# pzimbrod/fem-glass-tempering

Measured on AMD Instinct MI355X. Metric: DOF-updates/sec (coupled thermo-visco time step, 3D CG1 hex), higher is better.
Workload: dtype f64; 1 GPU; C4 3D plate CG1/CG1 400x400x50 hex (8200851 T-dofs), dt 0.1, coupled 6-term Prony; parallelism=single GPU, one partition (no communication), output=none (reference writes VTX/XDMF every step), krylov_form=PETSc KSPCG, geometric-multigrid V-cycle preconditioner, preconditioner=gmg, visco_fields=state (T, Tf, Tf_partial, phi, xi, s_tilde, sigma_tilde, sigma)

## Files before the change

fem-glass-tempering_amd/csrc/tv_context.cpp:

```cpp
#include <cstdlib>

#include "tv_ctx.h"

namespace tv {

static std::mutex g_err_mu;
static std::string g_err;

void set_global_error(const std::string& m) {
  std::lock_guard<std::mutex> lk(g_err_mu);
  g_err = m;
}

void axis_coefs(const std::vector<double>& X, int first, int count, std::vector<double>& out) {
  const int n = (int)X.size();
  out.assign((size_t)count * C_NCOEF, 0.0);
  for (int q = 0; q < count; ++q) {
    const int i = first + q;
    double* c = &out[(size_t)q * C_NCOEF];
    if (n == 1) {
      c[C_MDI] = 1.0;
      continue;
    }
    const double hlo = (i > 0) ? X[i] - X[i - 1] : 0.0;
// ... 1098 lines not shown
    output_release(c->out, set);
    return c->fail(TV_ERR_HIP, std::string("output gather: ") + hipGetErrorString(e));
  }
  std::string err;
  if (!output_submit(c->out, set, t, c->stream, err)) return c->fail(TV_ERR_STATE, "output: " + err);
  return TV_OK;
}


int tv_output_close(void* ctx) {
  Ctx* c = static_cast<Ctx*>(ctx);
  if (!c) return TV_ERR_ARG;
  if (!c->out) return TV_OK;
  hipSetDevice(c->device);
  const std::string e = output_destroy(c->out);
  c->out = nullptr;
  c->out_fields.clear();
  if (!e.empty()) return c->fail(TV_ERR_STATE, "output: " + e);
  return TV_OK;
}


int tv_set_dirichlet(void* ctx, int enable, double value) {
  Ctx* c = static_cast<Ctx*>(ctx);
  if (!c) return TV_ERR_ARG;
  if (c->O.model_mode != TV_MODEL_PAPER)
    return c->fail(TV_ERR_STATE, "Dirichlet condition: only with model_mode = TV_MODEL_PAPER (the reference's "
                                 "own path cannot run, ThermoViscoProblem.py:236-243)");
  if (enable && c->amg_on)
    return c->fail(TV_ERR_STATE, "Dirichlet condition: not with TV_PC_AMG (Jacobi or the box multigrid)");
  hipSetDevice(c->device);
  c->dir_on = enable != 0;
  c->dir_value = value;
  if (c->dir_on && c->fam_T == TV_CG && !c->dB) {
    const size_t nb = sizeof(double) * (size_t)std::max<int64_t>(1, c->nT);
    HIPC(tv_dev_alloc(&c->dB, nb, kMemDoubles));
    HIPC(tv_dev_alloc(&c->dtmp, nb, kMemDoubles));
    HIPC(hipMemsetAsync(c->dtmp, 0, nb, c->stream));
    HIPC(hipStreamSynchronize(c->stream));
  }
  return TV_OK;
}


int tv_sync(void* ctx) {
  Ctx* c = static_cast<Ctx*>(ctx);
  if (!c) return TV_ERR_ARG;
  HIPC(hipStreamSynchronize(c->stream));
  return TV_OK;
}


int tv_get_options(void* ctx, tv_options* out) {
  Ctx* c = static_cast<Ctx*>(ctx);
  if (!c || !out) return TV_ERR_ARG;
  *out = c->O;
  return TV_OK;
}


int tv_set_newton_tolerances(void* ctx, double rtol, double atol, int max_it, int error_on_nonconvergence) {
  Ctx* c = static_cast<Ctx*>(ctx);
  if (!c) return TV_ERR_ARG;
  if (!(rtol >= 0.0) || !(atol >= 0.0) || max_it < 1)
    return c->fail(TV_ERR_ARG, "Newton tolerances: rtol >= 0, atol >= 0 and max_it >= 1");
  c->O.newton_rtol = rtol;
// ... 21 lines not shown
```

fem-glass-tempering_amd/csrc/tv_ctx.h:

```cpp
#pragma once
#include <rccl/rccl.h>

#include <algorithm>
#include <array>
#include <cmath>
#include <cstdio>
#include <cstring>
#include <memory>
#include <mutex>
#include <string>
#include <vector>

#include "tv_internal.h"

namespace tv {

struct FieldInfo {
  double* ptr = nullptr;
  void* base = nullptr;
  int bs = 1;
  int space = 0;
  bool alloc = false;
};

struct MgLevel {
  CgGrid g{};
  std::vector<double> X[3];
  int64_t n = 0;
  double omega = 0.0;
  double *T = nullptr, *b = nullptr, *x = nullptr, *w = nullptr, *dinv = nullptr;
  MgXfer xf{};
  double* coef[3] = {nullptr, nullptr, nullptr};
  int64_t* bnodes = nullptr;
  double* ffbuf[2] = {nullptr, nullptr};
  std::vector<void*> bufs;
  bool dinv_interior = false;
  bool dist = false;
  int first2 = 0;
  int inj0 = 0, inj1 = 0;
  double* mask = nullptr;
  RRArgs rr{};
};

struct AmgLevel {
  int64_t n = 0;
  Sell A, P, R;
  UmGrid sg{};
  bool geo0 = false;
  int64_t gfine[3] = {0, 0, 0}, gcoarse[3] = {0, 0, 0};
  int64_t a_nnz = 0, p_nnz = 0, r_nnz = 0;
  double omega = 0.0;
  double *dinv = nullptr, *b = nullptr, *x = nullptr, *w = nullptr;
};

struct Ctx {
  std::string err;
  int device = 0;
  hipStream_t stream = nullptr;
  hipEvent_t ev0 = nullptr, ev1 = nullptr;
  hipEvent_t evp[2] = {nullptr, nullptr};
  hipEvent_t evn[2] = {nullptr, nullptr};
  const double* nrm_dev = nullptr;
  double* ngate = nullptr;
  const double* gate_dev = nullptr;
  const double* solve_gate = nullptr;
  int newton_slot = 0;
  bool newton_first = true;
  bool newton_ahead = true;
  tv_params P{};
  tv_options O{};
  int dim = 1;
  int fam_T = TV_CG, fam_S = TV_CG;
  int perm[3] = {0, -1, -1};
  int n_parts = 1, part = 0;
// ... 152 lines not shown
int allreduce(Ctx* c, double* v, int n);
int reduce_logic(Ctx* c, int n, int W, int kind, int check_done);
int cgs_raxis(const Ctx* c);
int cgs_exchange(Ctx* c, double* wout, const double* fout);
int require_comm(Ctx* c, const char* what);
int refresh_dirty_ghosts(Ctx* c);

void op_residual(Ctx* c, const double* T, const double* Tp, double* F);
void op_diag(Ctx* c, const double* T, double* d, int invert);
void op_japply(Ctx* c, const double* T, const double* x, double* y, double* partials, int* np);
bool op_japply_fused(Ctx* c, const double* T, int* np, const RedTail* tail = nullptr, int it = 0);
PcgState pcg_state_init(const Ctx* c);
int ts_flush(Ctx* c);
CgsBuffers cgs_buffers(Ctx* c, const double* T, int it);
int newton(Ctx* c, int* out_its, int* out_kits, int* out_conv, int step_end = 0, bool* end_queued = nullptr);
int visco(Ctx* c, bool copy_Tprev, const NewtonGate& gate = NewtonGate{});
int queue_newton_norm(Ctx* c, const double* nrm2);
int publish(Ctx* c, void* host_dst, const void* dev_src, size_t bytes);
void launch_bc_mask(Ctx* c, double* dinv);

int mg_setup(Ctx* c);
int mg_prepare(Ctx* c, const double* T);
int mg_dg_weight(Ctx* c, const double* T);
int mg_apply0(Ctx* c, const double* T, const RedTail* tail);
int pcg_solve_mg(Ctx* c, const double* T, int* its, int* reason, bool post = false);
bool mg_next_level(const std::vector<double> (&Xp)[3], double da, bool automatic, std::vector<double> (&Xc)[3],
                   std::vector<char> (&is_c)[3], int coarse[3]);
void mg_axis_tables(const std::vector<double>& Xf, const std::vector<char>& is_c, std::vector<int>& pi,
                    std::vector<double>& pw, std::vector<int>& ri, std::vector<double>& rw);
int mg_level_vectors(Ctx* c, MgLevel& L);
double mg_gershgorin(const std::vector<double> (&X)[3], double dt_alpha);
double mg_omega(double b);
int mg_level(Ctx* c, size_t l);
template <class T>
int mg_upload(Ctx* c, MgLevel& L, const std::vector<T>& h, const T** out) {
  void* p = nullptr;
  HIPC(tv_dev_alloc(&p, sizeof(T) * std::max<size_t>(1, h.size()), mem_kind<T>()));
  L.bufs.push_back(p);
  HIPC(hipMemcpy(p, h.data(), sizeof(T) * h.size(), hipMemcpyHostToDevice));
  *out = static_cast<const T*>(p);
  return TV_OK;
}

int mg_setup_dist(Ctx* c);
int pcg_solve_mg_dist(Ctx* c, const double* T, int* its, int* reason, bool post = false);
int mg_prepare_dist(Ctx* c, const double* T);
void fine_window(const Ctx* c, int64_t* off, int64_t* n);
int mg_apply0_dist(Ctx* c, const double* T, const RedTail* tail);

}
```

fem-glass-tempering_amd/csrc/tv_internal.h:

```cpp
#pragma once
#include <hip/hip_runtime.h>
#include <cstdint>
#include <string>
#include <type_traits>
#include <vector>

#include "tvfem.h"

namespace tv {

constexpr int kWave = 64;
constexpr int kSeg = kWave - 2;
constexpr int kBlock = 256;

enum { kMemDoubles = 0, kMemOther = 1 };
template <class T>
constexpr int mem_kind() {
  return std::is_same<T, double>::value ? kMemDoubles : kMemOther;
}
hipError_t tv_dev_alloc(void** p, size_t bytes, int kind);
hipError_t tv_dev_free(void* p);
template <class T>
inline hipError_t tv_dev_alloc(T** p, size_t bytes, int kind) {
  void* q = nullptr;
// ... 303 lines not shown
  const double* rw[3];
  int aligned;
};
void launch_mg_restrict(const MgXfer& x, const PcgState* st, const double* bf, const double* wf, const FaceAdd* fa,
                        const double* mask, double* bc, const double* dinv_c, double omega_c, double* xc,
                        hipStream_t s);
struct RRAxis {
  const int* f0;
  const double* w;
};
struct RRArgs {
  int on;
  int fn[3], cn[3];
  RRAxis ax[3];
  double da;
  int raxis, nseg, qchunk;
};
constexpr int kRRQMaxChunk = 64;
bool launch_mg_rrestrict(const RRArgs& a, const PcgState* st, const double* b, const double* x, const FaceAdd& fa,
                         double* bc, const double* dinv_c, double omega_c, double* xc, hipStream_t s);
void launch_cg_facet_faces(const CgGrid& g, const double* T, const double* x, const PcgState* st, hipStream_t s);
FaceAdd cg_face_add_all(const CgGrid& g);

struct CoarsePost {
  const double* b;
  const double* w;
  const double* dinv;
  double omega;
  FaceAdd fa;
};
void launch_mg_prolong(const MgXfer& x, const PcgState* st, double* xf, const double* xc, const double* mask,
                       hipStream_t s, const CoarsePost* cp = nullptr);
bool mg_prolong_smooths(const MgXfer& x);
bool mg_restrict_folds_faces(const MgXfer& x);
void launch_mg_jacobi(int64_t n, const PcgState* st, const double* b, const double* w, const FaceAdd* fa,
                      const double* dinv, double omega, double* x, int mode, hipStream_t s);
void launch_mg_inject(const MgXfer& x, const double* Tf, double* Tc, hipStream_t s);
void launch_mg_inject_range(const MgXfer& x, const double* Tf, double* Tc, int k0, int k1, hipStream_t s);
void launch_mg_resid(int64_t n, const PcgState* st, const double* b, double* w, const FaceAdd* fa, const double* mask,
                     hipStream_t s);
void launch_mg_ownmask(int64_t n, int64_t own0, int64_t own1, const double* dinv, double* mask, hipStream_t s);
constexpr int kMgPrepMax = 4;
struct MgPrep {
  int nlev;
  const double* Tbase;
  MgXfer xf[kMgPrepMax];
  double* T[kMgPrepMax];
  double* dinv[kMgPrepMax];
  CgGrid g[kMgPrepMax];
  int64_t off_n[kMgPrepMax + 1];
  int64_t off_b[kMgPrepMax + 1];
};
void launch_mg_prepare(const MgPrep& p, hipStream_t s);
bool cg_uses_march(const CgGrid& g);
void launch_mg_dg_restrict(const DgGrid& g, const PcgState* st, const double* bf, const double* wf, const double* mask,
                           double* bc, const double* dinv_c, double omega_c, double* xc, int kg0, hipStream_t s);
void launch_mg_dg_prolong(const DgGrid& g, const PcgState* st, double* xf, const double* xc, const double* mask,
                          int kg0, hipStream_t s);
void launch_mg_dg_T(const DgGrid& g, const double* Tdg, double* Tcg, int kg0, hipStream_t s);
int launch_mg_pow(int64_t n, const double* dinv, double* y, double* partials, hipStream_t s);
void launch_mg_scale(int64_t n, const double* y, double a, double* x, hipStream_t s);
bool launch_cg_japply_tail(const CgGrid& g, const double* T, const double* x, double* y, const PcgState* st,
                           double* partials, const RedTail* tail, hipStream_t s);
void launch_cg_japply_partial(const CgGrid& g, const double* T, const double* x, double* y, const PcgState* st,
                              hipStream_t s);
void launch_mg_update(int64_t n, const PcgState* st, const double* pA, const double* pB, const double* w,
                      const FaceAdd* fa, const double* dinv, double omega, double* r, double* dx, double* x0,
                      int it_host, int init, hipStream_t s, const double* lag = nullptr,
                      unsigned* counter = nullptr);
void launch_mg_update_cgs(int64_t n, const PcgState* st, const double* u, double* s, const double* z, double* p,
                          double* dx, double* r, const double* dinv, double omega, double* x0, bool first,
                          const double* lag, int lag_kind, unsigned* counter, hipStream_t stream);
int launch_cg_japply_post(const CgGrid& g, const double* T, const double* x, const double* r, const double* dinv,
                          double omega, double* z, const PcgState* st, double* partials, const RedTail* tail,
                          hipStream_t s);
int launch_mg_post(int64_t n, const PcgState* st, const double* x0, const double* r, const double* w,
                   const FaceAdd* fa, const double* dinv, double omega, double* z, double* partials,
                   const RedTail* tail, hipStream_t s);

void launch_pcg_update(int64_t n, PcgState* st, const double* pA, const double* pB, const double* w,
                       const double* dinv, double* dx, double* z, double* partials, hipStream_t s,
                       const RedTail* tail = nullptr, const FaceAdd* fa = nullptr, int it_host = 0);
void launch_pcg_dx_tail(int64_t n, const PcgState* st, const double* pA, const double* pB, double* dx, int its,
                        hipStream_t s);
void launch_mg_dx_finish(int64_t n, const PcgState* st, const double* pA, const double* pB, double* dx, int its,
                         hipStream_t s);
void launch_reduce_logic(const double* partials, int n, int W, double* out, PcgState* st, int kind,
// ... 27 lines not shown
```

fem-glass-tempering_amd/csrc/tv_measure.cpp:

```cpp
#include <algorithm>

#include "tv_ctx.h"

namespace tv {
__global__ __launch_bounds__(kBlock) void k_read_sweep(const double* __restrict__ a, int64_t n, double* out) {
  double acc = 0.0;
  for (int64_t t = blockIdx.x * (int64_t)kBlock + threadIdx.x; t < n; t += (int64_t)gridDim.x * kBlock) acc += a[t];
  if (acc == 12345.678) out[blockIdx.x] = acc;
}
__global__ void k_spin(uint64_t ticks) {
  if (threadIdx.x == 0) {
    const uint64_t t0 = __builtin_amdgcn_s_memrealtime();
    while (__builtin_amdgcn_s_memrealtime() - t0 < ticks) __builtin_amdgcn_s_sleep(16);
  }
}
__global__ void k_noop() {}

}

using namespace tv;

extern "C" {

int tv_kernel_bytes(void* ctx, int kernel, double* bytes) {
// ... 14 lines not shown
      double per = 8.0 * (2 + 6 + tilde)
                   + 8.0 * (6 + 3 + tilde + dd);
      if (c->O.materialize) per += 8.0 * (2 + 3 * dd + 4 * 6 * dd);
      *bytes = per * n;
      break;
    }
    case 2:
      *bytes = 24.0 * n;
      break;
    case 3:
      *bytes = (c->cgs ? 88.0 : 32.0) * n;
      break;
    case 5:
    case 7:
      *bytes = 32.0 * n;
      break;
    case 4:
      *bytes = c->cgs ? 0.0 : 48.0 * n;
      break;
    case 6:
    case 8:
      *bytes = 48.0 * n;
      break;
    case 11: {
      if (!c->mg_on) return c->fail(TV_ERR_ARG, "kernel 11: preconditioner GMG not enabled");
      if (c->amg_on) {
        *bytes = amg_cycle_bytes(c);
        break;
      }
      const bool rr0 = !c->mg_dg && !c->mg.empty() && c->mg[0].rr.on;
      double b = (c->mg_dg ? 16.0 + 16 + 16 + 16 + 32 : (rr0 ? 0.0 : 16.0) + 16 + 16 + 24) * n;
      for (size_t l = 0; l < c->mg.size(); ++l) {
        const double nl = (double)c->mg[l].n;
        b += 24.0 * nl;
        const bool rr = l + 1 < c->mg.size() && c->mg[l + 1].rr.on;
        if (l + 1 < c->mg.size())
          b += ((rr ? 0.0 : 16.0) + 16 + 16 + 16 + 24) * nl;
      }
      *bytes = b;
      break;
    }
    default:
      return c->fail(TV_ERR_ARG, "unknown kernel id");
  }
  return TV_OK;
}


int tv_time_kernel(void* ctx, int kernel, int reps, double* ms) {
  Ctx* c = static_cast<Ctx*>(ctx);
  if (!c || !ms || reps < 1) return TV_ERR_ARG;
  hipSetDevice(c->device);
  if (kernel == 4 && c->cgs) return c->fail(TV_ERR_ARG, "kernel 4: no separate update in the single-reduction PCG");
  if (kernel >= 3 && kernel <= 8) {
    PcgState h{};
    h.beta = 1.0; h.betaold = 2.0; h.a = 1e-3; h.it = 1; h.done = 0; h.max_it = 1 << 30;
    h.gamma = 1.0; h.eta = 1.0;
    HIPC(hipMemcpyAsync(c->st, &h, sizeof(PcgState), hipMemcpyHostToDevice, c->stream));
  }
  int upd_it = 0;
  if (c->um && (kernel == 0 || kernel == 10)) launch_um_robin_fold(c->umg, c->f[TV_F_T].ptr, c->stream);
  auto jx = [&]() {
    if (c->um) launch_um_japply(c->umg, c->f[TV_F_T].ptr, c->pA, c->w, c->stream);
    else op_japply(c, c->f[TV_F_T].ptr, c->pA, c->w, nullptr, nullptr);
  };
  if (kernel == 11) {
// ... 217 lines not shown
```

fem-glass-tempering_amd/csrc/tv_mgdist.cpp:

```cpp
#include "tv_ctx.h"

namespace tv {

constexpr int64_t kMgReplicateNodes = 300000;

namespace {

std::vector<int> owners_level0(int N2, int P) {
  std::vector<int> own((size_t)N2, 0);
  for (int p = 0; p < P; ++p) {
    int b0, b1;
    part_planes(N2, P, p, &b0, &b1);
    for (int k = b0; k < b1; ++k) own[(size_t)k] = p;
  }
  return own;
}

void owned_range(const std::vector<int>& own, int p, int* lo, int* hi) {
  *lo = *hi = 0;
  bool found = false;
  for (size_t k = 0; k < own.size(); ++k)
    if (own[k] == p) {
      if (!found) *lo = (int)k;
      found = true;
// ... 225 lines not shown
    if (!local && l - 1 < A) {
      const int skip = std::max(0, gdep(l - 1) - need(l - 1));
      x.f_kb = p > 0 ? skip : 0;
      x.f_ke = p < P - 1 ? x.fn[2] - skip : x.fn[2];
    }
    if (Lv.dist) {
      x.c_kb = Lv.g.k_begin;
      x.c_ke = Lv.g.k_end;
      x.aligned = 0;
    } else if (l == A) {
      (void)reach_lo;
      (void)reach_hi;
      x.c_kb = 0;
      x.c_ke = x.cn[2];
      x.aligned = 0;
    } else {
      x.c_kb = 0;
      x.c_ke = x.cn[2];
      x.aligned = 1;
    }
  }
  if (A < L) {
    const LevelRef r = level_ref(c, (size_t)(A - 1), nullptr);
    const int64_t nloc = (int64_t)r.g->n0 * r.g->n1 * r.g->n2;
    double** m = (A - 1 == 0) ? &c->mg_mask0 : &c->mg[A - 2].mask;
    HIPC(tv_dev_alloc(m, sizeof(double) * (size_t)std::max<int64_t>(1, nloc), kMemDoubles));
    launch_mg_ownmask(nloc, r.off, r.off + r.n_own, nullptr, *m, c->stream);
    HIPC(hipGetLastError());
  }
  if (c->mg_cgs) {
    HIPC(tv_dev_alloc(&c->mg_s, sizeof(double) * (size_t)std::max<int64_t>(1, c->nT), kMemDoubles));
    HIPC(hipMemsetAsync(c->mg_s, 0, sizeof(double) * (size_t)std::max<int64_t>(1, c->nT), c->stream));
  }
  c->mg_on = true;
  return TV_OK;
}

int mg_prepare_dist(Ctx* c, const double* T) {
  if (c->mg_dg) return mg_prepare(c, T);
  const double* Tf = T;
  for (size_t l = 1; l <= c->mg.size(); ++l) {
    MgLevel& L = c->mg[l - 1];
    if (L.dist) {
      launch_mg_inject_range(L.xf, Tf, L.T, L.inj0, L.inj1, c->stream);
      if (int e = halo_grid(c, L.g, L.T)) return e;
    } else if ((int)l == c->mg_A) {
      HIPC(hipMemsetAsync(L.T, 0, sizeof(double) * (size_t)L.n, c->stream));
      launch_mg_inject_range(L.xf, Tf, L.T, L.inj0, L.inj1, c->stream);
      if (int e = allreduce_vec(c, L.T, L.n)) return e;
    } else {
      launch_mg_inject(L.xf, Tf, L.T, c->stream);
    }
    launch_cg_diag(L.g, L.T, L.dinv, 1, c->stream, L.dinv_interior);
    L.dinv_interior = true;
    Tf = L.T;
  }
  HIPC(hipGetLastError());
  return TV_OK;
}

int mg_apply0_dist(Ctx* c, const double* T, const RedTail* tail) {
  if (c->amg_on || c->mg_dg) {
    const int r = c->amg_on ? amg_apply0(c, tail) : mg_apply0(c, T, tail);
    return r < 0 ? -r : TV_OK;
  }
  hipStream_t s = c->stream;
  const size_t L = c->mg.size() + 1;
  const size_t A = (size_t)c->mg_A;
  const double* dmask = c->dir_on ? c->dinv : nullptr;
  const size_t ldown = std::min(A, L);
  auto vhalo = [&](const CgGrid& g, double* v) -> int { return c->mg_local ? TV_OK : halo_grid(c, g, v); };
  const bool deep = c->ghost_depth > 1;
  for (size_t l = 0; l < ldown; ++l) {
    const LevelRef r = level_ref(c, l, T);
    if (!(deep && l == 0))
      if (int e = vhalo(*r.g, r.x)) return e;
    if (l + 1 == L) break;
    launch_cg_japply_partial(*r.g, r.T, r.x, r.w, c->st, s);
    FaceAdd fa = cg_face_add(*r.g, r.woff);
    MgLevel& C = c->mg[l];
    if (l + 1 < A) {
      launch_mg_resid(r.n_win, c->st, r.b + r.woff, r.w + r.woff, &fa, l == 0 && dmask ? dmask + r.woff : nullptr, s);
      if (!(deep && l == 0))
        if (int e = vhalo(*r.g, r.w)) return e;
      launch_mg_restrict(C.xf, c->st, r.w, nullptr, nullptr, nullptr, C.b, C.dinv, C.omega, C.x, s);
    } else {
      const double* mask = (l == 0) ? c->mg_mask0 : c->mg[l - 1].mask;
      const FaceAdd fa0 = cg_face_add(*r.g, 0);
      launch_mg_restrict(C.xf, c->st, r.b, r.w, &fa0, mask, C.b, nullptr, 0.0, nullptr, s);
// ... 252 lines not shown
```

fem-glass-tempering_amd/csrc/tv_mgsolve.cpp:

```cpp
#include <cstdlib>

#include "tv_ctx.h"

namespace tv {
constexpr int64_t kMgFoldFacesNodes = 4000000;

double mg_gershgorin(const std::vector<double> (&X)[3], double dt_alpha) {
  using Row = std::array<double, 6>;
  std::vector<Row> rows[3];
  for (int s = 0; s < 3; ++s) {
    std::vector<double> cf;
    axis_coefs(X[s], 0, (int)X[s].size(), cf);
    for (size_t i = 0; i < X[s].size(); ++i) {
      const double* c = &cf[i * C_NCOEF];
      rows[s].push_back({c[C_MLO], c[C_MDI], c[C_MUP], c[C_KLO], c[C_KDI], c[C_KUP]});
    }
    std::sort(rows[s].begin(), rows[s].end());
    rows[s].erase(std::unique(rows[s].begin(), rows[s].end()), rows[s].end());
  }
  double b = 0.0;
  for (const Row& r0 : rows[0])
    for (const Row& r1 : rows[1])
      for (const Row& r2 : rows[2]) {
        double sum = 0.0, diag = 0.0;
// ... 211 lines not shown
  const int64_t rowblocks = (x.cn[a.raxis] + 7) / 8;
  a.qchunk = std::min(x.cn[qa], kRRQMaxChunk);
  while ((int64_t)a.nseg * rowblocks * ((x.cn[qa] + a.qchunk - 1) / a.qchunk) < target && a.qchunk > 3)
    a.qchunk = (a.qchunk + 1) / 2;
  if (a.qchunk < 1 || a.qchunk > kRRQMaxChunk)
    return c->fail(TV_ERR_STATE, "GMG: fused residual restriction: march chunk " + std::to_string(a.qchunk) +
                                     " outside [1, " + std::to_string(kRRQMaxChunk) + "]");
  a.on = 1;
  return TV_OK;
}

constexpr int64_t kRRMinNodes = 3000000;
static unsigned rr_levels(int64_t fine_nodes) {
  const char* e = std::getenv("TVFEM_MG_RR");
  if (e) return (unsigned)std::strtoul(e, nullptr, 0);
  return fine_nodes >= kRRMinNodes ? 1u : 0u;
}

int mg_level_vectors(Ctx* c, MgLevel& L) {
  const CgGrid& f = c->cg;
  L.g.dt = f.dt; L.g.dt_alpha = f.dt_alpha; L.g.dt_f = f.dt_f;
  L.g.a_rad = f.a_rad; L.g.a_conv = f.a_conv; L.g.T_amb = f.T_amb; L.g.T_amb4 = f.T_amb4;
  L.n = (int64_t)L.g.n0 * L.g.n1 * L.g.n2;
  for (double** q : {&L.T, &L.b, &L.x, &L.w, &L.dinv}) {
    void* p = nullptr;
    HIPC(tv_dev_alloc(&p, sizeof(double) * (size_t)std::max<int64_t>(1, L.n), kMemDoubles));
    HIPC(hipMemsetAsync(p, 0, sizeof(double) * (size_t)std::max<int64_t>(1, L.n), c->stream));
    L.bufs.push_back(p);
    *q = static_cast<double*>(p);
  }
  return TV_OK;
}

int mg_setup(Ctx* c) {
  const bool dg = c->fam_T == TV_DG;
  if (c->dim != 3 || c->um || (!dg && !cg_cgs_supported(c->cg)) || (dg && (c->dg.deg1 || c->dg.deg2)))
    return c->fail(TV_ERR_ARG, "preconditioner GMG: 3D CG1 or DG1 temperature space on a rectilinear mesh only");
  if (c->cgs) return c->fail(TV_ERR_ARG, "preconditioner GMG runs in the KSPCG form (pcg_variant KSPCG or AUTO)");
  if (c->n_parts > 1 && !dg) return mg_setup_dist(c);
  if (c->n_parts > 1) c->mg_A = 1;
  std::vector<double> tmp, Xf[3];
  for (int s = 0; s < 3; ++s) Xf[s] = storage_coords(c, s, tmp);
  const double da = c->P.dt * c->P.alpha;
  HIPC(tv_dev_alloc(&c->mgx, sizeof(double) * (size_t)std::max<int64_t>(1, c->nT), kMemDoubles));
  HIPC(hipMemsetAsync(c->mgx, 0, sizeof(double) * (size_t)std::max<int64_t>(1, c->nT), c->stream));
  if (dg) {
    c->mg_dg = true;
    HIPC(tv_dev_alloc(&c->dggface, sizeof(double) * (size_t)dg_gface_size(c->dg), kMemDoubles));
    c->mg_omega0 = 0.0;
    if (int e = mg_add_cg_level(c, Xf, da)) return e;
  } else {
    c->mg_omega0 = mg_omega(mg_gershgorin(Xf, da));
  }
  const int max_levels = c->O.mg_levels > 0 ? c->O.mg_levels : 8;
  const bool automatic = c->O.mg_levels <= 0;
  std::vector<double> Xp[3] = {Xf[0], Xf[1], Xf[2]};
  for (int lev = 1 + (dg ? 1 : 0); lev < max_levels; ++lev) {
    std::vector<double> Xc[3];
    std::vector<char> is_c[3];
    int coarse[3];
    if (!mg_next_level(Xp, da, automatic, Xc, is_c, coarse)) break;
    c->mg.emplace_back();
    MgLevel& L = c->mg.back();
    for (int s = 0; s < 3; ++s) L.X[s] = Xc[s];
    if (int e = build_cg_grid(c, 3, L.X, 0, (int)L.X[2].size(), 0, 0, true, true, L.g, L.coef, &L.bnodes, L.ffbuf))
      return e;
    if (int e = mg_level_vectors(c, L)) return e;
    L.omega = mg_omega(mg_gershgorin(L.X, da));
    MgXfer& x = L.xf;
    std::vector<int> ri[3];
    std::vector<double> rw[3];
    for (int s = 0; s < 3; ++s) {
      std::vector<int> pi;
      std::vector<double> pw;
      mg_axis_tables(Xp[s], is_c[s], pi, pw, ri[s], rw[s]);
      if (int e = mg_upload(c, L, pi, &x.pi[s])) return e;
      if (int e = mg_upload(c, L, pw, &x.pw[s])) return e;
      if (int e = mg_upload(c, L, ri[s], &x.ri[s])) return e;
      if (int e = mg_upload(c, L, rw[s], &x.rw[s])) return e;
      x.fn[s] = (int)Xp[s].size();
      x.cn[s] = (int)L.X[s].size();
      x.coarse[s] = coarse[s];
    }
    x.f_kb = 0;
    x.f_ke = x.fn[2];
    x.c_kb = 0;
    x.c_ke = x.cn[2];
    x.aligned = 1;
    const size_t from = c->mg.size() - 1 - (dg ? 1 : 0);
    if (!dg && ((rr_levels(c->nT) >> from) & 1u))
      if (int e = rr_setup(c, L, Xp, ri, rw)) return e;
    for (int s = 0; s < 3; ++s) Xp[s] = L.X[s];
  }
  c->mg_on = true;
  return TV_OK;
}


int mg_prepare(Ctx* c, const double* T) {
  if (c->amg_on) return TV_OK;
  const bool dgpart = c->mg_dg && c->n_parts > 1;
  auto dg_T = [&](MgLevel& L) -> int {
    if (!dgpart) {
      launch_mg_dg_T(c->dg, T, L.T, 0, c->stream);
      return TV_OK;
    }
    HIPC(hipMemsetAsync(L.T, 0, sizeof(double) * (size_t)L.n, c->stream));
    launch_mg_dg_T(c->dg, T, L.T, c->plane_begin - c->dg.k_begin, c->stream);
    return allreduce_vec(c, L.T, L.n);
  };
  const size_t base = c->mg_dg ? 1 : 0;
  const size_t ncg = c->mg.size() - std::min(c->mg.size(), base);
  bool ready = ncg > 0 && ncg <= (size_t)kMgPrepMax;
  for (size_t l = base; l < c->mg.size() && ready; ++l)
    ready = c->mg[l].dinv_interior && cg_uses_march(c->mg[l].g) && c->mg[l].g.bnodes != nullptr;
  if (ready) {
    if (base == 1) {
      MgLevel& L = c->mg[0];
      if (int e = dg_T(L)) return e;
      if (c->dggface) launch_dg_gface(c->dg, T, c->dggface, c->stream);
      launch_cg_diag(L.g, L.T, L.dinv, 1, c->stream, true);
    }
    MgPrep p{};
    p.nlev = (int)ncg;
    p.Tbase = base == 1 ? c->mg[0].T : T;
    for (size_t i = 0; i < ncg; ++i) {
      MgLevel& L = c->mg[base + i];
      p.xf[i] = L.xf;
      p.T[i] = L.T;
      p.dinv[i] = L.dinv;
      p.g[i] = L.g;
      p.off_n[i + 1] = p.off_n[i] + (L.n + 63) / 64 * 64;
      p.off_b[i + 1] = p.off_b[i] + (L.g.n_bnodes + 63) / 64 * 64;
    }
    launch_mg_prepare(p, c->stream);
    return TV_OK;
  }
  const double* Tf = T;
  for (size_t l = 0; l < c->mg.size(); ++l) {
    MgLevel& L = c->mg[l];
    if (l == 0 && c->mg_dg) {
      if (int e = dg_T(L)) return e;
      if (c->dggface) launch_dg_gface(c->dg, T, c->dggface, c->stream);
    }
    else launch_mg_inject(L.xf, Tf, L.T, c->stream);
    launch_cg_diag(L.g, L.T, L.dinv, 1, c->stream, L.dinv_interior);
    L.dinv_interior = true;
    Tf = L.T;
  }
  return TV_OK;
}

void mg_prolong_from(Ctx* c, size_t ci, double* xf, const double* mask) {
  MgLevel& C = c->mg[ci];
  const bool smoothed = ci + 1 < c->mg.size() && mg_prolong_smooths(C.xf);
  if (smoothed) {
    const CoarsePost cp{C.b, C.w, C.dinv, C.omega, cg_face_add(C.g, 0)};
    launch_mg_prolong(C.xf, c->st, xf, C.x, mask, c->stream, &cp);
  } else {
    launch_mg_prolong(C.xf, c->st, xf, C.x, mask, c->stream);
  }
}

static const char kRRChunkMsg[] = "GMG: fused residual restriction refused (march chunk out of range)";

int mg_level(Ctx* c, size_t l) {
  MgLevel& L = c->mg[l - 1];
  hipStream_t s = c->stream;
  if (l < c->mg.size()) {
    const MgLevel& C = c->mg[l];
    const FaceAdd fa = cg_face_add(L.g, 0);
    if (C.rr.on && fa.on) {
      launch_cg_facet_faces(L.g, L.T, L.x, c->st, s);
      if (!launch_mg_rrestrict(C.rr, c->st, L.b, L.x, cg_face_add_all(L.g), C.b, C.dinv, C.omega, C.x, s))
        return c->fail(TV_ERR_STATE, kRRChunkMsg);
    } else if (fa.on && mg_restrict_folds_faces(C.xf)) {
      launch_cg_japply_partial(L.g, L.T, L.x, L.w, c->st, s);
      launch_mg_restrict(C.xf, c->st, L.b, L.w, &fa, nullptr, C.b, C.dinv, C.omega, C.x, s);
    } else {
      launch_cg_japply(L.g, L.T, L.x, L.w, nullptr, nullptr, s, c->st);
      launch_mg_restrict(C.xf, c->st, L.b, L.w, nullptr, nullptr, C.b, C.dinv, C.omega, C.x, s);
    }
    if (int e = mg_level(c, l + 1)) return e;
    mg_prolong_from(c, l, L.x, nullptr);
    launch_cg_japply_partial(L.g, L.T, L.x, L.w, c->st, s);
    if (!mg_prolong_smooths(L.xf))
      launch_mg_jacobi(L.n, c->st, L.b, L.w, &fa, L.dinv, L.omega, L.x, 1, s);
  }
  return TV_OK;
}

int mg_apply0(Ctx* c, const double* T, const RedTail* tail) {
  if (c->amg_on) return amg_apply0(c, tail);
  const int64_t n = c->nT;
  hipStream_t s = c->stream;
  const double* mask = c->dir_on ? c->dinv : nullptr;
  if (c->mg_dg) {
    const DgGrid& d = c->dg;
    MgLevel& C = c->mg[0];
    if (c->n_parts > 1) {
      const int kg0 = c->plane_begin - d.k_begin;
// ... 200 lines not shown
```

Before: 846.2 million DOF-updates/s.

## Fuse the last two multigrid levels into one LDS-resident tail kernel

Adds a single kernel that handles the second-coarsest GMG level and the coarsest level together. Per tile it runs a pre-smooth, residual, restriction, coarse Jacobi, prolongation and post-smooth entirely in shared memory, with halos and precomputed boundary facet weights. This replaces several launches and global round trips at the bottom of the V-cycle. The cost is redundant halo work, a large LDS footprint per block that can limit occupancy, and an extra facet-weight precompute in the prepare step.

```diff
diff --git a/fem-glass-tempering_amd/csrc/tv_context.cpp b/fem-glass-tempering_amd/csrc/tv_context.cpp
--- a/fem-glass-tempering_amd/csrc/tv_context.cpp
+++ b/fem-glass-tempering_amd/csrc/tv_context.cpp
@@ -1154,6 +1154,8 @@
   hipSetDevice(c->device);
   c->dir_on = enable != 0;
   c->dir_value = value;
+  if (c->mg_on)
+    if (int e = mg_tail_plan(c)) return e;
   if (c->dir_on && c->fam_T == TV_CG && !c->dB) {
     const size_t nb = sizeof(double) * (size_t)std::max<int64_t>(1, c->nT);
     HIPC(tv_dev_alloc(&c->dB, nb, kMemDoubles));
diff --git a/fem-glass-tempering_amd/csrc/tv_ctx.h b/fem-glass-tempering_amd/csrc/tv_ctx.h
--- a/fem-glass-tempering_amd/csrc/tv_ctx.h
+++ b/fem-glass-tempering_amd/csrc/tv_ctx.h
@@ -40,6 +40,10 @@
   int inj0 = 0, inj1 = 0;
   double* mask = nullptr;
   RRArgs rr{};
+  bool tail = false;
+  int tail_axis = 2;
+  double* tail_w = nullptr;
+  bool x_smoothed = false;
 };
 
 struct AmgLevel {
@@ -258,6 +262,8 @@
 double mg_gershgorin(const std::vector<double> (&X)[3], double dt_alpha);
 double mg_omega(double b);
 int mg_level(Ctx* c, size_t l);
+int mg_tail_plan(Ctx* c);
+void mg_tail_prepare(Ctx* c);
 template <class T>
 int mg_upload(Ctx* c, MgLevel& L, const std::vector<T>& h, const T** out) {
   void* p = nullptr;
diff --git a/fem-glass-tempering_amd/csrc/tv_internal.h b/fem-glass-tempering_amd/csrc/tv_internal.h
--- a/fem-glass-tempering_amd/csrc/tv_internal.h
+++ b/fem-glass-tempering_amd/csrc/tv_internal.h
@@ -359,6 +359,7 @@
 void launch_mg_prolong(const MgXfer& x, const PcgState* st, double* xf, const double* xc, const double* mask,
                        hipStream_t s, const CoarsePost* cp = nullptr);
 bool mg_prolong_smooths(const MgXfer& x);
+bool mg_prolong_blocks(const MgXfer& x);
 bool mg_restrict_folds_faces(const MgXfer& x);
 void launch_mg_jacobi(int64_t n, const PcgState* st, const double* b, const double* w, const FaceAdd* fa,
                       const double* dinv, double omega, double* x, int mode, hipStream_t s);
@@ -380,6 +381,24 @@
 };
 void launch_mg_prepare(const MgPrep& p, hipStream_t s);
 bool cg_uses_march(const CgGrid& g);
+struct MgTailArgs {
+  CgGrid g;
+  MgXfer xf;
+  const PcgState* st;
+  const double* T;
+  const double* b;
+  const double* dinv;
+  const double* dinv_c;
+  double* x;
+  double* facew;
+  double omega, omega_c;
+  int64_t sy, sz, csy, csz;
+};
+constexpr int kMgTailTile = 8;
+bool mg_tail_fits(int axis, const CgGrid& g, const MgXfer& xf);
+int64_t mg_tail_facew_size(const CgGrid& g);
+void launch_mg_tail_facew(const MgTailArgs& a, int axis, hipStream_t s);
+void launch_mg_tail(const MgTailArgs& a, int axis, hipStream_t s);
 void launch_mg_dg_restrict(const DgGrid& g, const PcgState* st, const double* bf, const double* wf, const double* mask,
                            double* bc, const double* dinv_c, double omega_c, double* xc, int kg0, hipStream_t s);
 void launch_mg_dg_prolong(const DgGrid& g, const PcgState* st, double* xf, const double* xc, const double* mask,
diff --git a/fem-glass-tempering_amd/csrc/tv_measure.cpp b/fem-glass-tempering_amd/csrc/tv_measure.cpp
--- a/fem-glass-tempering_amd/csrc/tv_measure.cpp
+++ b/fem-glass-tempering_amd/csrc/tv_measure.cpp
@@ -70,6 +70,14 @@
       double b = (c->mg_dg ? 16.0 + 16 + 16 + 16 + 32 : (rr0 ? 0.0 : 16.0) + 16 + 16 + 24) * n;
       for (size_t l = 0; l < c->mg.size(); ++l) {
         const double nl = (double)c->mg[l].n;
+        if (c->mg[l].tail) {
+          b += 24.0 * nl + 24.0 * nl;
+          continue;
+        }
+        if (l > 0 && c->mg[l - 1].tail) {
+          b += 8.0 * nl;
+          continue;
+        }
         b += 24.0 * nl;
         const bool rr = l + 1 < c->mg.size() && c->mg[l + 1].rr.on;
         if (l + 1 < c->mg.size())
diff --git a/fem-glass-tempering_amd/csrc/tv_mgdist.cpp b/fem-glass-tempering_amd/csrc/tv_mgdist.cpp
--- a/fem-glass-tempering_amd/csrc/tv_mgdist.cpp
+++ b/fem-glass-tempering_amd/csrc/tv_mgdist.cpp
@@ -281,6 +281,7 @@
     HIPC(tv_dev_alloc(&c->mg_s, sizeof(double) * (size_t)std::max<int64_t>(1, c->nT), kMemDoubles));
     HIPC(hipMemsetAsync(c->mg_s, 0, sizeof(double) * (size_t)std::max<int64_t>(1, c->nT), c->stream));
   }
+  if (int e = mg_tail_plan(c)) return e;
   c->mg_on = true;
   return TV_OK;
 }
@@ -304,6 +305,7 @@
     L.dinv_interior = true;
     Tf = L.T;
   }
+  mg_tail_prepare(c);
   HIPC(hipGetLastError());
   return TV_OK;
 }
diff --git a/fem-glass-tempering_amd/csrc/tv_mgsolve.cpp b/fem-glass-tempering_amd/csrc/tv_mgsolve.cpp
--- a/fem-glass-tempering_amd/csrc/tv_mgsolve.cpp
+++ b/fem-glass-tempering_amd/csrc/tv_mgsolve.cpp
@@ -267,6 +267,43 @@
   return TV_OK;
 }
 
+int mg_tail_plan(Ctx* c) {
+  if (c->mg.size() < 2) return TV_OK;
+  MgLevel& U = c->mg[c->mg.size() - 2];
+  const MgLevel& C = c->mg.back();
+  U.tail = false;
+  U.x_smoothed = false;
+  const char* e = std::getenv("TVFEM_MG_TAIL");
+  if (e && std::atoi(e) == 0) return TV_OK;
+  const bool whole = !U.dist && !C.dist && C.xf.aligned;
+  int axis = U.g.n1 < U.g.n2 ? 1 : 2;
+  if (!mg_tail_fits(axis, U.g, C.xf)) axis = 3 - axis;
+  const bool ok = whole && cg_uses_march(U.g) && cg_uses_march(C.g) && mg_restrict_folds_faces(C.xf) &&
+                  mg_prolong_blocks(C.xf) && !c->dir_on && mg_tail_fits(axis, U.g, C.xf);
+  if (!ok) return TV_OK;
+  if (!U.tail_w) {
+    const size_t nb = sizeof(double) * (size_t)mg_tail_facew_size(U.g);
+    HIPC(tv_dev_alloc(&U.tail_w, nb, kMemDoubles));
+    HIPC(hipMemsetAsync(U.tail_w, 0, nb, c->stream));
+    U.bufs.push_back(U.tail_w);
+  }
+  U.tail = true;
+  U.tail_axis = axis;
+  U.x_smoothed = true;
+  return TV_OK;
+}
+
+static MgTailArgs tail_args(Ctx* c) {
+  const MgLevel& U = c->mg[c->mg.size() - 2];
+  const MgLevel& C = c->mg.back();
+  return MgTailArgs{U.g, C.xf, c->st, U.T, U.b, U.dinv, C.dinv, U.x, U.tail_w, U.omega, C.omega, 0, 0, 0, 0};
+}
+
+void mg_tail_prepare(Ctx* c) {
+  if (c->mg.size() < 2 || !c->mg[c->mg.size() - 2].tail) return;
+  launch_mg_tail_facew(tail_args(c), c->mg[c->mg.size() - 2].tail_axis, c->stream);
+}
+
 int mg_setup(Ctx* c) {
   const bool dg = c->fam_T == TV_DG;
   if (c->dim != 3 || c->um || (!dg && !cg_cgs_supported(c->cg)) || (dg && (c->dg.deg1 || c->dg.deg2)))
@@ -327,6 +364,7 @@
       if (int e = rr_setup(c, L, Xp, ri, rw)) return e;
     for (int s = 0; s < 3; ++s) Xp[s] = L.X[s];
   }
+  if (int e = mg_tail_plan(c)) return e;
   c->mg_on = true;
   return TV_OK;
 }
@@ -369,6 +407,7 @@
       p.off_b[i + 1] = p.off_b[i] + (L.g.n_bnodes + 63) / 64 * 64;
     }
     launch_mg_prepare(p, c->stream);
+    mg_tail_prepare(c);
     return TV_OK;
   }
   const double* Tf = T;
@@ -383,12 +422,13 @@
     L.dinv_interior = true;
     Tf = L.T;
   }
+  mg_tail_prepare(c);
   return TV_OK;
 }
 
 void mg_prolong_from(Ctx* c, size_t ci, double* xf, const double* mask) {
   MgLevel& C = c->mg[ci];
-  const bool smoothed = ci + 1 < c->mg.size() && mg_prolong_smooths(C.xf);
+  const bool smoothed = ci + 1 < c->mg.size() && mg_prolong_smooths(C.xf) && !C.x_smoothed;
   if (smoothed) {
     const CoarsePost cp{C.b, C.w, C.dinv, C.omega, cg_face_add(C.g, 0)};
     launch_mg_prolong(C.xf, c->st, xf, C.x, mask, c->stream, &cp);
@@ -402,6 +442,10 @@
 int mg_level(Ctx* c, size_t l) {
   MgLevel& L = c->mg[l - 1];
   hipStream_t s = c->stream;
+  if (L.tail) {
+    launch_mg_tail(tail_args(c), L.tail_axis, s);
+    return TV_OK;
+  }
   if (l < c->mg.size()) {
     const MgLevel& C = c->mg[l];
     const FaceAdd fa = cg_face_add(L.g, 0);
diff --git a/fem-glass-tempering_amd/csrc/tv_mgtail.hip b/fem-glass-tempering_amd/csrc/tv_mgtail.hip
--- /dev/null
+++ b/fem-glass-tempering_amd/csrc/tv_mgtail.hip
@@ -0,0 +1,443 @@
+#include <algorithm>
+
+#include "tv_stencil.h"
+
+namespace tv {
+namespace {
+
+constexpr int kTailHalo = 4;
+
+template <int TX, int NZ>
+struct TailPlan {
+  static constexpr int EM = TX + 2 * kTailHalo;
+  static constexpr int NT = EM * EM;
+  static constexpr int CM = EM / 2 + 1;
+  static constexpr int CNZ = NZ / 2 + 1;
+  static constexpr int kFine = NZ * EM * EM;
+  static constexpr int kCoarse = CNZ * CM * CM;
+  static constexpr int kCoef = (2 * EM + NZ) * C_NCOEF;
+  static constexpr int kRw = 3 * (2 * CM + CNZ);
+  static constexpr int kPw = 2 * (2 * EM + NZ);
+  static constexpr int kWs = 2 * NZ * EM * 9;
+  static constexpr size_t kBytes = sizeof(double) * (2 * kFine + kCoarse + kCoef + kRw + kPw + 2 * kWs);
+  static_assert(kBytes <= 160 * 1024, "the tail's LDS plan exceeds a gfx950 CU (160 KiB)");
+  static_assert(NT <= 1024 && NT % kWave == 0, "one thread per region column, whole waves");
+};
+
+__device__ __forceinline__ int clampi(int v, int lo, int hi) { return v < lo ? lo : (v > hi ? hi : v); }
+__device__ __forceinline__ int c_first(const MgXfer& x, int a, int f) {
+  return !x.coarse[a] ? f : min((f + 1) >> 1, x.cn[a] - 1);
+}
+__device__ __forceinline__ int c_last(const MgXfer& x, int a, int f) {
+  return !x.coarse[a] ? f : (f == x.fn[a] - 1 ? x.cn[a] - 1 : f >> 1);
+}
+__device__ __forceinline__ int c_centre(const MgXfer& x, int a, int I) {
+  return !x.coarse[a] ? I : (I == x.cn[a] - 1 ? x.fn[a] - 1 : 2 * I);
+}
+
+struct TailRegion {
+  int ex0, ey0, EX, EY, nz;
+  int64_t sy, sz;
+};
+
+template <int EM, int NZ, class Out>
+__device__ __forceinline__ void tail_march(const double* xs, const double* cf, const TailRegion& R, int tx, int ty,
+                                           double da, Out&& out) {
+  const double* cx = cf + tx * C_NCOEF;
+  const double* cy = cf + (EM + ty) * C_NCOEF;
+  double cA[3][3], cB[3][3];
+  int o[3][3];
+#pragma unroll
+  for (int b = 0; b < 3; ++b) {
+    const int yy = ty + b - 1;
+    const bool oky = yy >= 0 && yy < R.EY;
+    const double My = oky ? cy[C_MLO + b] : 0.0, Ky = oky ? cy[C_KLO + b] : 0.0;
+#pragma unroll
+    for (int a = 0; a < 3; ++a) {
+      const int xx = tx + a - 1;
+      const bool okx = xx >= 0 && xx < R.EX;
+      const double Mx = okx ? cx[C_MLO + a] : 0.0, Kx = okx ? cx[C_KLO + a] : 0.0;
+      cA[b][a] = My * Mx;
+      cB[b][a] = My * Kx + Ky * Mx;
+      o[b][a] = clampi(xx, 0, R.EX - 1) + EM * clampi(yy, 0, R.EY - 1);
+    }
+  }
+  auto plane_ab = [&](int k, double& A, double& B) {
+    const double* p = xs + EM * EM * k;
+    A = 0.0;
+    B = 0.0;
+#pragma unroll
+    for (int b = 0; b < 3; ++b)
+#pragma unroll
+      for (int a = 0; a < 3; ++a) {
+        const double v = p[o[b][a]];
+        A += cA[b][a] * v;
+        B += cB[b][a] * v;
+      }
+  };
+  double A0 = 0.0, B0 = 0.0, A1, B1, A2 = 0.0, B2 = 0.0;
+  plane_ab(0, A1, B1);
+#pragma unroll
+  for (int k = 0; k < NZ; ++k) {
+    if (k < R.nz) {
+      if (k + 1 < R.nz) {
+        plane_ab(k + 1, A2, B2);
+      } else {
+        A2 = 0.0;
+        B2 = 0.0;
+      }
+      const double* cz = cf + (2 * EM + k) * C_NCOEF;
+      const double y = cz[C_MLO] * (A0 + da * B0) + cz[C_MDI] * (A1 + da * B1) + cz[C_MUP] * (A2 + da * B2) +
+                       da * (cz[C_KLO] * A0 + cz[C_KDI] * A1 + cz[C_KUP] * A2);
+      out(k, y);
+      A0 = A1; B0 = B1;
+      A1 = A2; B1 = B2;
+    }
+  }
+}
+
+template <int TX, int NZ, int NZX>
+__global__ __launch_bounds__((TX + 2 * kTailHalo) * (TX + 2 * kTailHalo)) void k_mg_tail(MgTailArgs a) {
+  using P = TailPlan<TX, NZ>;
+  constexpr int EM = P::EM, CM = P::CM, NT = P::NT;
+  __shared__ double s_xs[P::kFine], s_rs[P::kFine], s_cs[P::kCoarse], s_cf[P::kCoef], s_rw[P::kRw], s_pw[P::kPw];
+  __shared__ double s_wy[P::kWs], s_wx[P::kWs];
+  const CgGrid& g = a.g;
+  const MgXfer& x = a.xf;
+  const int n0 = g.n0, n1 = g.n1, nz = NZX > 0 ? NZX : g.n2;
+  const int ntx = (n0 + TX - 1) / TX;
+  const int bx = (int)blockIdx.x % ntx, by = (int)blockIdx.x / ntx;
+  const int i0 = bx * TX, j0 = by * TX;
+  const int i1 = min(n0, i0 + TX), j1 = min(n1, j0 + TX);
+  const int ex0 = max(0, i0 - kTailHalo), ex1 = min(n0, i1 + kTailHalo);
+  const int ey0 = max(0, j0 - kTailHalo), ey1 = min(n1, j1 + kTailHalo);
+  const TailRegion R{ex0, ey0, ex1 - ex0, ey1 - ey0, nz, a.sy, a.sz};
+  const int c0[3] = {c_first(x, 0, ex0), c_first(x, 1, ey0), 0};
+  const int cN[3] = {c_last(x, 0, ex1 - 1) - c0[0] + 1, c_last(x, 1, ey1 - 1) - c0[1] + 1, x.cn[2]};
+  const int tid = (int)threadIdx.x;
+  const int tx = tid % EM, ty = tid / EM;
+  const bool col = tx < R.EX && ty < R.EY;
+  const int gi = ex0 + tx, gj = ey0 + ty;
+  const int64_t plane = a.sz;
+  const int64_t gcol = col ? gi + a.sy * gj : 0;
+  const int lcol = tx + EM * ty;
+
+  const int done = a.st != nullptr ? a.st->done : 0;
+  double bb[NZ], dd[NZ];
+#pragma unroll
+  for (int k = 0; k < NZ; ++k) {
+    const bool ok = col && k < nz;
+    bb[k] = ok ? a.b[gcol + plane * k] : 0.0;
+    dd[k] = ok ? a.dinv[gcol + plane * k] : 0.0;
+  }
+  const int sx = gi == 0 ? 0 : 1, sy = gj == 0 ? 0 : 1;
+  const bool onx = col && ((gi == 0 && g.bnd[0][0]) || (gi == n0 - 1 && g.bnd[0][1]));
+  const bool ony = col && ((gj == 0 && g.bnd[1][0]) || (gj == n1 - 1 && g.bnd[1][1]));
+  const bool zf0 = g.bnd[2][0] != 0, zf1 = g.bnd[2][1] != 0;
+  const int64_t wo_y = 18 * (int64_t)n0 * n1, wo_x = wo_y + 18 * (int64_t)n0 * nz;
+  double wz0[9], wz1[9];
+#pragma unroll
+  for (int e = 0; e < 9; ++e) {
+    wz0[e] = (col && zf0) ? a.facew[((int64_t)gj * n0 + gi) * 9 + e] : 0.0;
+    wz1[e] = (col && zf1) ? a.facew[((int64_t)(n1 + gj) * n0 + gi) * 9 + e] : 0.0;
+  }
+  const bool fs_on[4] = {g.bnd[1][0] && ey0 == 0, g.bnd[1][1] && ey1 == n1, g.bnd[0][0] && ex0 == 0,
+                         g.bnd[0][1] && ex1 == n0};
+  constexpr int KW = (NZ * EM * 9 + NT - 1) / NT;
+  double wv[4][KW];
+#pragma unroll
+  for (int fs = 0; fs < 4; ++fs) {
+    const int row = fs < 2 ? n0 : n1, first = fs < 2 ? ex0 : ey0, cnt = fs < 2 ? R.EX : R.EY;
+    const int64_t base = (fs < 2 ? wo_y : wo_x) + (int64_t)(fs & 1) * nz * row * 9;
+#pragma unroll
+    for (int q = 0; q < KW; ++q) {
+      const int t = tid + q * NT;
+      const int e = t % 9, l = (t / 9) % EM, k = t / (9 * EM);
+      wv[fs][q] = (fs_on[fs] && k < nz && l < cnt) ? a.facew[base + ((int64_t)k * row + first + l) * 9 + e] : 0.0;
+    }
+  }
+  constexpr int KC = (P::kCoarse + NT - 1) / NT;
+  double dc[KC];
+#pragma unroll
+  for (int q = 0; q < KC; ++q) {
+    const int t = tid + q * NT;
+    const int ci = t % CM, cj = (t / CM) % CM, ck = t / (CM * CM);
+    const bool ok = ci < cN[0] && cj < cN[1] && ck < cN[2];
+    dc[q] = ok ? a.dinv_c[(c0[0] + ci) + a.csy * (c0[1] + cj) + a.csz * ck] : 0.0;
+  }
+  constexpr int KF = (P::kCoef + NT - 1) / NT;
+  double cfv[KF];
+#pragma unroll
+  for (int q = 0; q < KF; ++q) {
+    const int t = tid + q * NT;
+    const int row = t / C_NCOEF, e = t % C_NCOEF;
+    const int ax = row < EM ? 0 : (row < 2 * EM ? 1 : 2);
+    const int loc = row - ax * EM;
+    const int first = ax == 0 ? ex0 : (ax == 1 ? ey0 : 0), cnt = ax == 0 ? R.EX : (ax == 1 ? R.EY : nz);
+    cfv[q] = (t < P::kCoef && loc < cnt) ? g.coef[ax][(int64_t)(first + loc) * C_NCOEF + e] : 0.0;
+  }
+  constexpr int KR = (P::kRw + NT - 1) / NT;
+  double rwv[KR];
+#pragma unroll
+  for (int q = 0; q < KR; ++q) {
+    const int t = tid + q * NT;
+    const int row = t / 3, e = t % 3;
+    const int ax = row < CM ? 0 : (row < 2 * CM ? 1 : 2);
+    const int loc = row - ax * CM;
+    rwv[q] = (t < P::kRw && loc < cN[ax]) ? x.rw[ax][3 * (c0[ax] + loc) + e] : 0.0;
+  }
+  constexpr int KP = (P::kPw + NT - 1) / NT;
+  double pwv[KP];
+#pragma unroll
+  for (int q = 0; q < KP; ++q) {
+    const int t = tid + q * NT;
+    const int row = t / 2, e = t % 2;
+    const int ax = row < EM ? 0 : (row < 2 * EM ? 1 : 2);
+    const int loc = row - ax * EM;
+    const int first = ax == 0 ? ex0 : (ax == 1 ? ey0 : 0), cnt = ax == 0 ? R.EX : (ax == 1 ? R.EY : nz);
+    pwv[q] = (t < P::kPw && loc < cnt) ? x.pw[ax][2 * (first + loc) + e] : 0.0;
+  }
+
+  if (done) return;
+
+  if (col) {
+#pragma unroll
+    for (int k = 0; k < NZ; ++k)
+      if (k < nz) {
+        s_rs[lcol + EM * EM * k] = bb[k];
+        s_xs[lcol + EM * EM * k] = a.omega * dd[k] * bb[k];
+      }
+  }
+#pragma unroll
+  for (int fs = 0; fs < 4; ++fs)
+    if (fs_on[fs]) {
+      double* dst = (fs < 2 ? s_wy : s_wx) + (fs & 1) * (NZ * EM * 9);
+#pragma unroll
+      for (int q = 0; q < KW; ++q)
+        if (tid + q * NT < NZ * EM * 9) dst[tid + q * NT] = wv[fs][q];
+    }
+#pragma unroll
+  for (int q = 0; q < KC; ++q)
+    if (tid + q * NT < P::kCoarse) s_cs[tid + q * NT] = dc[q];
+#pragma unroll
+  for (int q = 0; q < KF; ++q)
+    if (tid + q * NT < P::kCoef) s_cf[tid + q * NT] = cfv[q];
+#pragma unroll
+  for (int q = 0; q < KR; ++q)
+    if (tid + q * NT < P::kRw) s_rw[tid + q * NT] = rwv[q];
+#pragma unroll
+  for (int q = 0; q < KP; ++q)
+    if (tid + q * NT < P::kPw) s_pw[tid + q * NT] = pwv[q];
+  __syncthreads();
+
+  int pox[3], poy[3];
+#pragma unroll
+  for (int q = 0; q < 3; ++q) {
+    pox[q] = clampi(tx + q - 1, 0, R.EX - 1);
+    poy[q] = EM * clampi(ty + q - 1, 0, R.EY - 1);
+  }
+  auto facets = [&](int k) {
+    double f = 0.0;
+    if (k == 0 || k == nz - 1) {
+      const double* p = s_xs + EM * EM * k;
+#pragma unroll
+      for (int u = 0; u < 3; ++u)
+#pragma unroll
+        for (int v = 0; v < 3; ++v) {
+          const double xv = p[pox[u] + poy[v]];
+          if (k == 0) f += wz0[u * 3 + v] * xv;
+          if (k == nz - 1) f += wz1[u * 3 + v] * xv;
+        }
+    }
+    if (ony) {
+      const double* w = s_wy + ((sy * NZ + k) * EM + tx) * 9;
+#pragma unroll
+      for (int v = 0; v < 3; ++v) {
+        const double* p = s_xs + EM * EM * clampi(k + v - 1, 0, nz - 1) + EM * ty;
+#pragma unroll
+        for (int u = 0; u < 3; ++u) f += w[u * 3 + v] * p[pox[u]];
+      }
+    }
+    if (onx) {
+      const double* w = s_wx + ((sx * NZ + k) * EM + ty) * 9;
+#pragma unroll
+      for (int v = 0; v < 3; ++v) {
+        const double* p = s_xs + EM * EM * clampi(k + v - 1, 0, nz - 1) + tx;
+#pragma unroll
+        for (int u = 0; u < 3; ++u) f += w[u * 3 + v] * p[poy[u]];
+      }
+    }
+    return f;
+  };
+
+  if (col)
+    tail_march<EM, NZ>(s_xs, s_cf, R, tx, ty, g.dt_alpha,
+                       [&](int k, double y) { s_rs[lcol + EM * EM * k] = bb[k] - y - facets(k); });
+  __syncthreads();
+
+#pragma unroll
+  for (int q = 0; q < KC; ++q) {
+    const int t = tid + q * NT;
+    const int ci = t % CM, cj = (t / CM) % CM, ck = t / (CM * CM);
+    if (ci < cN[0] && cj < cN[1] && ck < cN[2]) {
+      const int fi = c_centre(x, 0, c0[0] + ci) - ex0, fj = c_centre(x, 1, c0[1] + cj) - ey0, fk = c_centre(x, 2, ck);
+      const double* wi = s_rw + 3 * ci;
+      const double* wj = s_rw + 3 * (CM + cj);
+      const double* wk = s_rw + 3 * (2 * CM + ck);
+      double acc = 0.0;
+#pragma unroll
+      for (int c = 0; c < 3; ++c) {
+        double pl = 0.0;
+#pragma unroll
+        for (int b = 0; b < 3; ++b) {
+          const int base = EM * (clampi(fj + b - 1, 0, R.EY - 1) + EM * clampi(fk + c - 1, 0, nz - 1));
+          double row = 0.0;
+#pragma unroll
+          for (int aa = 0; aa < 3; ++aa) row += wi[aa] * s_rs[base + clampi(fi + aa - 1, 0, R.EX - 1)];
+          pl += wj[b] * row;
+        }
+        acc += wk[c] * pl;
+      }
+      s_cs[t] = a.omega_c * s_cs[t] * acc;
+    }
+  }
+  __syncthreads();
+
+  const bool in1 = col && gi >= i0 - 1 && gi < i1 + 1 && gj >= j0 - 1 && gj < j1 + 1;
+  if (in1) {
+    int pa[2], pb[2];
+    pmap(x, 0, gi, pa[0], pa[1]);
+    pmap(x, 1, gj, pb[0], pb[1]);
+    const double* wi = s_pw + 2 * tx;
+    const double* wj = s_pw + 2 * (EM + ty);
+    int oc[2][2];
+    double wc[2][2];
+#pragma unroll
+    for (int b = 0; b < 2; ++b)
+#pragma unroll
+      for (int aa = 0; aa < 2; ++aa) {
+        oc[b][aa] = clampi(pa[aa] - c0[0], 0, cN[0] - 1) + CM * clampi(pb[b] - c0[1], 0, cN[1] - 1);
+        wc[b][aa] = wj[b] * wi[aa];
+      }
+#pragma unroll
+    for (int k = 0; k < NZ; ++k) {
+      if (k >= nz) break;
+      int pc[2];
+      pmap(x, 2, k, pc[0], pc[1]);
+      const double* wk = s_pw + 2 * (2 * EM + k);
+      double acc = 0.0;
+#pragma unroll
+      for (int c = 0; c < 2; ++c) {
+        const double* p = s_cs + CM * CM * pc[c];
+        acc += wk[c] * ((wc[0][0] * p[oc[0][0]] + wc[0][1] * p[oc[0][1]]) + (wc[1][0] * p[oc[1][0]] + wc[1][1] * p[oc[1][1]]));
+      }
+      s_xs[lcol + EM * EM * k] += acc;
+    }
+  }
+  __syncthreads();
+
+  const bool own = col && gi >= i0 && gi < i1 && gj >= j0 && gj < j1;
+  if (own) {
+    tail_march<EM, NZ>(s_xs, s_cf, R, tx, ty, g.dt_alpha, [&](int k, double y) {
+      const double r = bb[k] - y - facets(k);
+      a.x[gcol + plane * k] = s_xs[lcol + EM * EM * k] + a.omega * dd[k] * r;
+    });
+  }
+}
+
+__global__ __launch_bounds__(kBlock) void k_mg_tail_facew(MgTailArgs a) {
+  const CgGrid& g = a.g;
+  const int n[3] = {g.n0, g.n1, g.n2};
+  const int64_t gs[3] = {1, a.sy, a.sz};
+  const int64_t cnt[3] = {2 * (int64_t)n[0] * n[1], 2 * (int64_t)n[0] * n[2], 2 * (int64_t)n[1] * n[2]};
+  const int64_t t = blockIdx.x * (int64_t)blockDim.x + threadIdx.x;
+  if (t >= cnt[0] + cnt[1] + cnt[2]) return;
+  const int grp = t < cnt[0] ? 0 : (t < cnt[0] + cnt[1] ? 1 : 2);
+  const int64_t u0 = t - (grp > 0 ? cnt[0] : 0) - (grp > 1 ? cnt[1] : 0);
+  const int ax = 2 - grp;
+  const int t1 = (ax == 0) ? 1 : 0, t2 = (ax == 2) ? 1 : 2;
+  const int side = (int)(u0 / ((int64_t)n[t1] * n[t2]));
+  const int r = (int)(u0 - (int64_t)side * n[t1] * n[t2]);
+  const int c1 = r % n[t1], c2 = r / n[t1];
+  double* w = a.facew + t * 9;
+  if (!g.bnd[ax][side]) {
+    for (int e = 0; e < 9; ++e) w[e] = 0.0;
+    return;
+  }
+  const int64_t me = (side ? (int64_t)(n[ax] - 1) * gs[ax] : 0) + c1 * gs[t1] + c2 * gs[t2];
+  double Tp[3][3];
+#pragma unroll
+  for (int u = 0; u < 3; ++u)
+#pragma unroll
+    for (int v = 0; v < 3; ++v) {
+      const int p = c1 + u - 1, q = c2 + v - 1;
+      const bool ok = p >= 0 && p < n[t1] && q >= 0 && q < n[t2];
+      Tp[u][v] = ok ? a.T[me + (u - 1) * gs[t1] + (v - 1) * gs[t2]] : 0.0;
+    }
+  const double* h1 = g.coef[t1] + (int64_t)c1 * C_NCOEF;
+  const double* h2 = g.coef[t2] + (int64_t)c2 * C_NCOEF;
+  for (int e = 0; e < 9; ++e) {
+    double Pp[3][3];
+#pragma unroll
+    for (int u = 0; u < 3; ++u)
+#pragma unroll
+      for (int v = 0; v < 3; ++v) Pp[u][v] = (u * 3 + v == e) ? 1.0 : 0.0;
+    w[e] = facet_sum<MODE_JAC, false, false, false>(g, h1[C_HLO], h1[C_HHI], h2[C_HLO], h2[C_HHI], Tp, Pp);
+  }
+}
+
+constexpr int kTailNz = 16;
+constexpr int kTailNzExact = 14;
+
+MgTailArgs tail_axes(const MgTailArgs& in, int axis) {
+  MgTailArgs a = in;
+  a.sy = in.g.n0;
+  a.sz = (int64_t)in.g.n0 * in.g.n1;
+  a.csy = in.xf.cn[0];
+  a.csz = (int64_t)in.xf.cn[0] * in.xf.cn[1];
+  if (axis == 1) {
+    std::swap(a.sy, a.sz);
+    std::swap(a.csy, a.csz);
+    std::swap(a.g.n1, a.g.n2);
+    std::swap(a.g.coef[1], a.g.coef[2]);
+    for (int e = 0; e < 2; ++e) std::swap(a.g.bnd[1][e], a.g.bnd[2][e]);
+    std::swap(a.xf.fn[1], a.xf.fn[2]);
+    std::swap(a.xf.cn[1], a.xf.cn[2]);
+    std::swap(a.xf.coarse[1], a.xf.coarse[2]);
+    std::swap(a.xf.pi[1], a.xf.pi[2]);
+    std::swap(a.xf.pw[1], a.xf.pw[2]);
+    std::swap(a.xf.ri[1], a.xf.ri[2]);
+    std::swap(a.xf.rw[1], a.xf.rw[2]);
+  }
+  return a;
+}
+
+}
+
+bool mg_tail_fits(int axis, const CgGrid& g, const MgXfer& xf) {
+  if (axis != 1 && axis != 2) return false;
+  const int nz = axis == 2 ? g.n2 : g.n1;
+  return nz >= 2 && nz <= kTailNz && xf.cn[axis] <= kTailNz / 2 + 1 && xf.fn[0] == g.n0 && xf.fn[1] == g.n1 &&
+         xf.fn[2] == g.n2;
+}
+
+int64_t mg_tail_facew_size(const CgGrid& g) {
+  return 18 * ((int64_t)g.n0 * g.n1 + (int64_t)g.n0 * g.n2 + (int64_t)g.n1 * g.n2);
+}
+
+void launch_mg_tail_facew(const MgTailArgs& in, int axis, hipStream_t s) {
+  const MgTailArgs a = tail_axes(in, axis);
+  const int64_t n = mg_tail_facew_size(a.g) / 9;
+  hipLaunchKernelGGL(k_mg_tail_facew, dim3((unsigned)((n + kBlock - 1) / kBlock)), dim3(kBlock), 0, s, a);
+}
+
+void launch_mg_tail(const MgTailArgs& in, int axis, hipStream_t s) {
+  const MgTailArgs a = tail_axes(in, axis);
+  constexpr int TX = kMgTailTile;
+  const int ntx = (a.g.n0 + TX - 1) / TX, nty = (a.g.n1 + TX - 1) / TX;
+  const dim3 grid((unsigned)(ntx * nty)), block(TailPlan<TX, kTailNz>::NT);
+  if (a.g.n2 == kTailNzExact) hipLaunchKernelGGL((k_mg_tail<TX, kTailNz, kTailNzExact>), grid, block, 0, s, a);
+  else hipLaunchKernelGGL((k_mg_tail<TX, kTailNz, 0>), grid, block, 0, s, a);
+}
+
+}
```

Measured after the change: 855.1 million DOF-updates/s (median of 6 runs). 1.01x the previous value.
